# e-ago/CoMD-CUDA-Async

Hardware: AMD Instinct MI355X
Metric: atom_updates_per_sec (higher is better)
Workload: dtype f64

## Files before the change

### comd-cuda-async_amd/csrc/hip/comd_device.hip

```cpp
#include <hip/hip_runtime.h>
#include <cstdio>
#include <cstdlib>
#include <cstring>
#include <cmath>
#include <vector>
#include <map>
#include <utility>

#include "comd_hip.h"
#include "device_common.h"
#include "lj_kernels.h"
#include "lj_table_kernels.h"
#include "eam_kernels.h"
#include "step_kernels.h"
#include "nl_kernels.h"
#include "eam_brick_kernels.h"
#include "eam_atom_brick_kernels.h"
#include "virial_kernels.h"
#include "rdf_kernels.h"
#include "langevin_kernels.h"

static int g_rank = 0;

#define HIP_CHECK(cmd)                                                                                     \
   do {                                                                                                    \
      hipError_t status_ = (cmd);                                                                          \
      if (status_ != hipSuccess) {                                                                         \
         int dev_ = -1; (void)hipGetDevice(&dev_);                                                         \
         fprintf(stderr, "Rank %d, GPU: %d, Error in file %s at line %d\n", g_rank, dev_, __FILE__, __LINE__); \
         fprintf(stderr, "HIP error %d: %s\n", (int)status_, hipGetErrorString(status_));                  \
         exit(-1);                                                                                         \
      }                                                                                                    \
   } while (0)

#define LAUNCH_CHECK() HIP_CHECK(hipGetLastError())

static inline hipStream_t S(comdStream_t s) { return (hipStream_t)s; }
static inline int ceilDiv(long a, long b) { return (int)((a + b - 1) / b); }

static void allowDynamicLds(const void* fn, size_t lds)
{
   static std::map<std::pair<int, const void*>, size_t> granted;
   int dev = 0; HIP_CHECK(hipGetDevice(&dev));
   size_t& g = granted[std::make_pair(dev, fn)];
   if (lds > g) { HIP_CHECK(hipFuncSetAttribute(fn, hipFuncAttributeMaxDynamicSharedMemorySize, (int)lds)); g = lds; }
}

struct ComdTuning {
   bool   nlGlobal;
   bool   eamNlLds;
   int    ljWaves;
   bool   ljPrune;
   int    ljListCap;
   double ljListBudgetMb;
   bool   ljCtaSlabs;
   bool   eamCtaCell;
   bool   eamThreadAtomCell;
   bool   eamGroups;
   int    eamBrickBy, eamBrickBz;
   int    eamImage;
   int    eamAblate;
   bool   eamClamp;
   int    eamAtomRows;
   bool   eamAtomHandover;
   int    eamAtomBrickBy, eamAtomBrickBz;
   int    eamAtomLdsPad;
   int    eamCtaWaves;
   int    eamStencil;
   bool   nlSync;
   bool   eamListsEveryBuild;
   bool   nlBankOrder;
   double nlMargin;
};
static ComdTuning readTuning()
{
   auto env = getenv;
   auto num = [&](const char* name) { const char* e = env(name); return e ? atoi(e) : 0; };
   auto is = [&](const char* name, const char* value) { const char* e = env(name); return e && !strcmp(e, value); };
   auto isZero = [&](const char* name) { const char* e = env(name); return e && atoi(e) == 0; };
   auto shape = [&](const char* name, int* by, int* bz) { const char* e = env(name); if (!(e && sscanf(e, "%d,%d", by, bz) == 2 && *by >= 1 && *bz >= 1 && *by * *bz <= 64)) *by = *bz = 0; };
   ComdTuning t;
   t.nlGlobal = env("COMD_NL_GLOBAL") != nullptr;
   t.eamNlLds = is("COMD_EAM_NL", "lds");
   t.ljWaves = num("COMD_LJ_WAVES") > 0 ? num("COMD_LJ_WAVES") : 0;
   t.ljPrune = !isZero("COMD_LJ_PRUNE");
   t.ljListCap = num("COMD_LJ_LIST_CAP") > 0 ? (num("COMD_LJ_LIST_CAP") + 7) & ~7 : 0;
   t.ljListBudgetMb = env("COMD_LJ_LIST_BUDGET_MB") ? atof(env("COMD_LJ_LIST_BUDGET_MB")) : INFINITY;
   t.ljCtaSlabs = num("COMD_LJ_CTA_SLABS") != 0;
   t.eamCtaCell = is("COMD_EAM_CTA", "cell");
   t.eamThreadAtomCell = is("COMD_EAM_THREAD_ATOM", "cell");
   t.eamGroups = !isZero("COMD_EAM_GROUPS");
   shape("COMD_EAM_BRICK", &t.eamBrickBy, &t.eamBrickBz);
   t.eamImage = num("COMD_EAM_IMAGE") >= 64 ? (num("COMD_EAM_IMAGE") + 7) / 8 * 8 : 0;
   t.eamAblate = num("COMD_EAM_ABLATE");
   t.eamClamp = num("COMD_EAM_CLAMP") != 0;
   t.eamAtomRows = num("COMD_EAM_ATOM_ROWS") >= 8 && num("COMD_EAM_ATOM_ROWS") <= 128 ? num("COMD_EAM_ATOM_ROWS") / 8 * 8 : 0;
   t.eamAtomHandover = !isZero("COMD_EAM_ATOM_HANDOVER");
   shape("COMD_EAM_ATOM_BRICK", &t.eamAtomBrickBy, &t.eamAtomBrickBz);
   t.eamAtomLdsPad = num("COMD_EAM_ATOM_LDS_PAD");
   t.eamCtaWaves = num("COMD_EAM_CTA_WAVES") >= 1 && num("COMD_EAM_CTA_WAVES") <= 8 ? num("COMD_EAM_CTA_WAVES") : 0;
   t.eamStencil = num("COMD_EAM_STENCIL") >= 64 ? (num("COMD_EAM_STENCIL") + 7) / 8 * 8 : 0;
   t.nlSync = num("COMD_NL_SYNC") != 0;
   t.eamListsEveryBuild = env("COMD_EAM_LISTS_EVERY_BUILD") != nullptr;
   t.nlBankOrder = num("COMD_NL_BANK_ORDER") != 0;
   t.nlMargin = env("COMD_NL_MARGIN") && atof(env("COMD_NL_MARGIN")) >= 0.0 && atof(env("COMD_NL_MARGIN")) < 1.0 ? atof(env("COMD_NL_MARGIN")) : -1.0;
   return t;
}
static const ComdTuning& tuningOf(SimGpu* sim) { if (!sim->tuning) sim->tuning = new ComdTuning(readTuning()); return *(const ComdTuning*)sim->tuning; }
static double latticeConstantOf(const SimGpu* sim) { return sim->latticeConstant > 0.0 ? sim->latticeConstant : 3.615; }
static const double SPHERE_VOLUME = 4.18879020478639;


struct ForceTiming {
   struct Ev { hipEvent_t a, b; int kind; };
   std::vector<Ev> pool;
   size_t used = 0;
   double ms[2] = { 0.0, 0.0 };
   int launches[2] = { 0, 0 };
   bool on = false;
};

static void timingFlush(ForceTiming* t)
{
   if (!t) return;
   for (size_t i = 0; i < t->used; ++i) {
      float ms = 0.f;
      HIP_CHECK(hipEventSynchronize(t->pool[i].b));
      HIP_CHECK(hipEventElapsedTime(&ms, t->pool[i].a, t->pool[i].b));
      t->ms[t->pool[i].kind] += ms;
      t->launches[t->pool[i].kind] += 1;
   }
   t->used = 0;
}

struct ForceTimer {
   ForceTiming* t; hipStream_t st; int idx;
   ForceTimer(SimGpu* sim, hipStream_t s, int kind = 0) : t((ForceTiming*)sim->timing), st(s), idx(-1)
   {
// ... 368 lines not shown
{
   const size_t first = (size_t)sim->boxes.nLocalBoxes * sim->maxAtoms, slots = (size_t)(sim->boxes.nTotalBoxes - sim->boxes.nLocalBoxes) * sim->maxAtoms;
   const real_t* src[6] = { h->px, h->py, h->pz, h->rx, h->ry, h->rz };
   real_t* dst[6] = { sim->atoms.p.x, sim->atoms.p.y, sim->atoms.p.z, sim->atoms.r.x, sim->atoms.r.y, sim->atoms.r.z };
   for (int i = 0; i < 6; ++i) HIP_CHECK(hipMemcpy(dst[i] + first, src[i] + first, slots * sizeof(real_t), hipMemcpyHostToDevice));
   HIP_CHECK(hipMemcpy(sim->atoms.gid + first, h->gid + first, slots * sizeof(int), hipMemcpyHostToDevice));
   HIP_CHECK(hipMemcpy(sim->atoms.iSpecies + first, h->iSpecies + first, slots * sizeof(int), hipMemcpyHostToDevice));
}

extern "C" void updateNAtomsGpu(SimGpu* sim, const int* nAtomsHost)
{
   HIP_CHECK(hipMemcpy(sim->boxes.nAtoms, nAtomsHost, (size_t)sim->boxes.nTotalBoxes * sizeof(int), hipMemcpyHostToDevice));
}

extern "C" int compactHaloCells(const HostAtoms* h, int nLocalBoxes, int nTotalBoxes, int maxAtoms, char* h_compactAtoms, int* h_cellOffset)
{
   const int nHalo = nTotalBoxes - nLocalBoxes;
   h_cellOffset[0] = 0;
   for (int i = 0; i < nHalo; ++i) h_cellOffset[i + 1] = h_cellOffset[i] + h->nAtoms[nLocalBoxes + i];
   const int n = h_cellOffset[nHalo];
   int* gid = (int*)h_compactAtoms; int* type = gid + n;
   real_t* m = (real_t*)(type + n);
   for (int i = 0; i < nHalo; ++i) {
      size_t o = (size_t)(nLocalBoxes + i) * maxAtoms;
      for (int k = h_cellOffset[i]; k < h_cellOffset[i + 1]; ++k, ++o) {
         gid[k] = h->gid[o]; type[k] = h->iSpecies[o];
         m[k] = h->rx[o]; m[(size_t)n + k] = h->ry[o]; m[2 * (size_t)n + k] = h->rz[o];
         m[3 * (size_t)n + k] = h->px[o]; m[4 * (size_t)n + k] = h->py[o]; m[5 * (size_t)n + k] = h->pz[o];
      }
   }
   return n;
}

extern "C" void DestroyGpu(SimGpu* sim)
{
   HIP_CHECK(hipDeviceSynchronize());
   if (sim->timing) {
      ForceTiming* t = (ForceTiming*)sim->timing;
      timingFlush(t);
      for (auto& ev : t->pool) { (void)hipEventDestroy(ev.a); (void)hipEventDestroy(ev.b); }
      delete t;
   }
   delete (ComdTuning*)sim->tuning;
   void* ptrs[] = { sim->boxes.nAtoms, sim->atoms.r.x, sim->atoms.r.y, sim->atoms.r.z, sim->atoms.p.x, sim->atoms.p.y, sim->atoms.p.z,
                    sim->atoms.f.x, sim->atoms.f.y, sim->atoms.f.z, sim->atoms.e, sim->atoms.iSpecies, sim->atoms.gid,
                    sim->neighbor_cells, sim->species_mass, sim->eam_pot.phi.values, sim->eam_pot.rho.values, sim->eam_pot.f.values,
                    sim->eam_pot.rhobar, sim->eam_pot.dfEmbed, sim->nAtomsPrev, sim->cellDirty, sim->cellArrivals, sim->d_updateLinkCellsRequired, sim->status, sim->reduceBuf,
                    sim->boundary_cells, sim->interior_cells, sim->boundary1_cells,
                    sim->atoms.neighborList.list, sim->atoms.neighborList.nNeighbors, sim->atoms.neighborList.lastR.x,
                    sim->atoms.neighborList.lastR.y, sim->atoms.neighborList.lastR.z,
                    sim->atoms.neighborList.list16, sim->atoms.neighborList.stats, sim->atoms.neighborList.pairlist,
                    sim->boxes.boxIDLookUp, sim->boxes.boxIDLookUpReverse, sim->eam_pot.phiS.coefficients, sim->eam_pot.rhoS.coefficients,
                    sim->eam_pot.pairRows, sim->eam_pot.pairRowCount, sim->eam_pot.cellSel, sim->eam_pot.brickGroup, sim->eam_pot.brickList, sim->eam_pot.brickSel, sim->eam_pot.brickStats, sim->eam_pot.atomRows, sim->eam_pot.atomRowCount, sim->eam_pot.atomBrickSel,
                    sim->atoms.neighborList.brickRows, sim->atoms.neighborList.brickRowCount, sim->adapterScan, sim->lj_pot.waveCand, sim->lj_pot.waveCandCount, sim->lj_pot.packedR[0], sim->lj_pot.packedR[1], sim->lj_pot.packedF[0], sim->lj_pot.packedF[1],
                    sim->lj_pot.lj_interpolation.values, sim->virialBuf, sim->pairHistBuf };
   for (void* p : ptrs) if (p) HIP_CHECK(hipFree(p));
   if (sim->statusEvent) (void)hipEventDestroy((hipEvent_t)sim->statusEvent);
   if (sim->pinned) HIP_CHECK(hipHostFree(sim->pinned));
   if (sim->atoms.neighborList.updateRequiredHost) HIP_CHECK(hipHostFree(sim->atoms.neighborList.updateRequiredHost));
   if (sim->atoms.neighborList.brickStatsMirror) HIP_CHECK(hipHostFree(sim->atoms.neighborList.brickStatsMirror));
   if (sim->atoms.neighborList.brickStatsEvent) (void)hipEventDestroy((hipEvent_t)sim->atoms.neighborList.brickStatsEvent);
   if (sim->boundary_stream) HIP_CHECK(hipStreamDestroy(S(sim->boundary_stream)));
   if (sim->interior_stream) HIP_CHECK(hipStreamDestroy(S(sim->interior_stream)));
   memset(sim, 0, sizeof(*sim));
}

extern "C" void emptyHaloCellsGpu(SimGpu* sim, comdStream_t stream)
{
   const int nHalo = sim->boxes.nTotalBoxes - sim->boxes.nLocalBoxes;
   HIP_CHECK(hipMemsetAsync(sim->boxes.nAtoms + sim->boxes.nLocalBoxes, 0, (size_t)nHalo * sizeof(int), S(stream)));
}

extern "C" void comdCheckStatus(SimGpu* sim, const char* where)
{
   int st[4];
   HIP_CHECK(hipDeviceSynchronize());
   HIP_CHECK(hipMemcpy(st, sim->status, sizeof st, hipMemcpyDeviceToHost));
   if (st[0] | st[1] | st[2] | st[3]) {
      fprintf(stderr, "Rank %d, GPU: %d, %s: ", g_rank, sim->deviceId, where);
      if (st[0] & 1) fprintf(stderr, "a link cell overflowed its %d slots (raise --maxAtoms); ", sim->maxAtoms);
      if (st[0] & 2) fprintf(stderr, "a cell stencil holds more atoms than the cta_cell kernel can stage; ");
      if (st[1])     fprintf(stderr, "an atom moved beyond the halo region and was lost; ");
      if (st[2])     fprintf(stderr, "a halo message overflowed its buffer, or grew by more than 12.5 %% + 64 atoms in one step (COMD_HALO_HANDSHAKE=1 exchanges exact sizes); ");
      if (st[3] & 1) fprintf(stderr, "an atom has more neighbours inside the cutoff than a row of the EAM cta_cell kernel holds (1.5 x the FCC count; use -m thread_atom); ");
      if (st[3] & 2) fprintf(stderr, "an atom has more than %d neighbours inside cutoff + skin (raise --maxNeighbors); ", sim->atoms.neighborList.maxNeighbors);
      if (st[3] & 4) fprintf(stderr, "eamForce3Gpu[Async] covered the cells with another partition than eamForce1Gpu[Async] (include/comd_hip.h: same lists in both passes); ");
      fprintf(stderr, "\n");
      exit(-1);
   }
}

extern "C" void comdPollStatus(SimGpu* sim, comdStream_t stream, const char* where)
{
   int* mirror = (int*)(sim->pinned + 32);
   if (sim->statusMirrored) {
      sim->statusMirrored = 0;
      if (mirror[0] | mirror[1] | mirror[2] | mirror[3]) comdCheckStatus(sim, where);
      return;
   }
   if (sim->statusEvent) {
      if (hipEventQuery((hipEvent_t)sim->statusEvent) != hipSuccess) return;
      if (mirror[0] | mirror[1] | mirror[2] | mirror[3]) comdCheckStatus(sim, where);
   } else {
      hipEvent_t e; HIP_CHECK(hipEventCreateWithFlags(&e, hipEventDisableTiming)); sim->statusEvent = (void*)e;
   }
   HIP_CHECK(hipMemcpyAsync(mirror, sim->status, 4 * sizeof(int), hipMemcpyDeviceToHost, S(stream)));
   HIP_CHECK(hipEventRecord((hipEvent_t)sim->statusEvent, S(stream)));
}

extern "C" int comdReadDeviceInt(const int* d_ptr, comdStream_t stream)
{
   int v = 0;
   HIP_CHECK(hipMemcpyAsync(&v, d_ptr, sizeof(int), hipMemcpyDeviceToHost, S(stream)));
   HIP_CHECK(hipStreamSynchronize(S(stream)));
   return v;
}

static NlView nlView(SimGpu* sim)
{
   NeighborListGpu* n = &sim->atoms.neighborList;
   if (!n->list && !n->list16) { fprintf(stderr, "the *_nl methods need Verlet lists: allocate with GpuConfig.skinDistance > 0\n"); exit(-1); }
   if (n->nBuilds == 0) { fprintf(stderr, "the *_nl methods need buildNeighborListGpu before the first force call\n"); exit(-1); }
   NlView v; v.list = n->list; v.count = n->nNeighbors; v.maxNbr = n->maxNeighbors;
   return v;
}

static LjArgs makeLjArgs(SimGpu* sim, int num_cells, int* cells_list)
{
   LjArgs a;
   a.rx = sim->atoms.r.x; a.ry = sim->atoms.r.y; a.rz = sim->atoms.r.z;
   a.fx = sim->atoms.f.x; a.fy = sim->atoms.f.y; a.fz = sim->atoms.f.z; a.e = sim->atoms.e;
   a.nAtoms = sim->boxes.nAtoms; a.nbr = sim->neighbor_cells; a.cells = cells_list;
   a.nCells = num_cells; a.cap = sim->maxAtoms;
   const double sigma = sim->lj_pot.sigma, rc = sim->lj_pot.cutoff;
   a.rc2 = rc * rc;
   a.s6 = sigma * sigma * sigma * sigma * sigma * sigma;
   a.s6x2 = 2.0 * (sigma * sigma * sigma * sigma * sigma * sigma);
   const double rc6 = a.s6 / (a.rc2 * a.rc2 * a.rc2);
   a.eShift = rc6 * (rc6 - 1.0);
   a.eps = sim->lj_pot.epsilon;
   return a;
}

extern "C" void comdSetEnergyNeeded(SimGpu* sim, int on) { sim->needEnergy = on; }

static void ljBoxMargins(const SimGpu* sim, real_t rc2, real_t* rc2Box, real_t* grow)
{
   const double rel = sizeof(real_t) == 8 ? 1e-12 : 1e-5, eps = sizeof(real_t) == 8 ? 2.220446049250313e-16 : 1.1920929e-07;
   double big = 0.0;
   for (int a = 0; a < 3; ++a) {
      const double cellW = 1.0 / sim->boxes.invBoxSize[a];
      const double lo = fabs((double)sim->boxes.localMin[a] - cellW), hi = fabs((double)sim->boxes.localMax[a] + cellW);
      if (lo > big) big = lo;
      if (hi > big) big = hi;
   }
   const double rc = sqrt((double)rc2) * (1.0 + rel) + 8.0 * 1.7320508 * eps * big;
   *rc2Box = (real_t)(rc * rc);
   *grow = (real_t)(1.0 + rel);
}

static void ljBoxMarginsF(const SimGpu* sim, real_t rc2, float* rc2Box, float* grow)
{
   const double rel = 1e-5, eps = 1.1920929e-07;
   double big = 0.0;
   for (int a = 0; a < 3; ++a) {
      const double ext = (double)sim->boxes.localMax[a] - (double)sim->boxes.localMin[a] + 2.0 / sim->boxes.invBoxSize[a];
      if (ext > big) big = ext;
   }
   const double rc = sqrt((double)rc2) * (1.0 + rel) + 8.0 * 1.7320508 * eps * big;
   *rc2Box = (float)(rc * rc * (1.0 + 2.0 * eps));
   *grow = (float)(1.0 + rel);
}

struct LjThreadAtomLaunch { int w, wavesPerBlock; unsigned nBlocks; bool prune; LjWaveLists wl; };

static LjThreadAtomLaunch prepareLjThreadAtom(SimGpu* sim, const LjArgs& a, int num_cells, int* cells_list, comdStream_t stream)
{
   int w = sim->maxAtoms / 64;
   if (sim->max_atoms_cell > 0 && (sim->max_atoms_cell + 16 + 63) / 64 < w) w = (sim->max_atoms_cell + 16 + 63) / 64;
   const ComdTuning& tune = tuningOf(sim);
   if (tune.ljWaves && tune.ljWaves < w) w = tune.ljWaves;
   const int wavesPerBlock = w <= 4 ? w : 4;
   const unsigned nBlocks = w <= 4 ? (unsigned)num_cells : (unsigned)ceilDiv((long)num_cells * w, 4);
   const bool pruneEnv = tune.ljPrune;
   LjPotentialGpu* lj = &sim->lj_pot;
   if (pruneEnv && !lj->waveCand && lj->packedCap == 0) {
      std::vector<int> counts((size_t)sim->boxes.nTotalBoxes);
      HIP_CHECK(hipMemcpyAsync(counts.data(), sim->boxes.nAtoms, counts.size() * sizeof(int), hipMemcpyDeviceToHost, S(stream)));
      HIP_CHECK(hipStreamSynchronize(S(stream)));
      int fullest = sim->max_atoms_cell;
      for (int c : counts) if (c > fullest) fullest = c;
      const int occ = fullest + 16 < sim->maxAtoms ? fullest + 16 : sim->maxAtoms;
      lj->waveCandWaves = w;
      lj->waveCandCap = ((int)(0.70 * 27 * occ) + 7) & ~7;
      if (tune.ljListCap) lj->waveCandCap = tune.ljListCap;
      lj->packedCap = ((occ + 7) & ~7) < sim->maxAtoms ? ((occ + 7) & ~7) : sim->maxAtoms;
      const double listBytes = (double)sim->boxes.nLocalBoxes * lj->waveCandWaves * lj->waveCandCap * 4.0 + (double)sim->boxes.nLocalBoxes * lj->waveCandWaves * 8.0
                               + (sim->interior_stream ? 2.0 : 1.0) * (double)sim->boxes.nTotalBoxes * lj->packedCap * (sizeof(LjPos4) + sizeof(float4));
      size_t freeB = 0, totalB = 0;
      HIP_CHECK(hipMemGetInfo(&freeB, &totalB));
      if ((double)sim->boxes.nTotalBoxes * lj->packedCap * sizeof(LjPos4) >= 4294967296.0) lj->packedCap = -1;
      else if (listBytes + 2.0e9 > (double)freeB || listBytes > 1.0e6 * tune.ljListBudgetMb) {
         fprintf(stderr, "Rank %d: LJ candidate lists need %.1f GB, %.1f GB are free: running without them (the plain 27-cell walk, ~1.4x slower)\n",
                 g_rank, listBytes / 1e9, (double)freeB / 1e9);
         lj->packedCap = -1;
      } else {
         auto tryAlloc = [](size_t bytes) { void* p = nullptr; if (hipMalloc(&p, bytes ? bytes : 8) != hipSuccess) { (void)hipGetLastError(); p = nullptr; } return p; };
         const size_t recs = (size_t)sim->boxes.nTotalBoxes * lj->packedCap * 4;
         lj->waveCand = (unsigned*)tryAlloc((size_t)sim->boxes.nLocalBoxes * lj->waveCandWaves * lj->waveCandCap * sizeof(unsigned));
         lj->waveCandCount = (int*)tryAlloc((size_t)sim->boxes.nLocalBoxes * lj->waveCandWaves * 2 * sizeof(int));
         bool ok = lj->waveCand && lj->waveCandCount;
         for (int k = 0; k < (sim->interior_stream ? 2 : 1) && ok; ++k) {
            lj->packedR[k] = (real_t*)tryAlloc(recs * sizeof(real_t));
            lj->packedF[k] = (float*)tryAlloc(recs * sizeof(float));
            ok = lj->packedR[k] && lj->packedF[k];
         }
         if (!ok) {
            void* ps[6] = { lj->waveCand, lj->waveCandCount, lj->packedR[0], lj->packedF[0], lj->packedR[1], lj->packedF[1] };
            for (void* q : ps) if (q) (void)hipFree(q);
            lj->waveCand = nullptr; lj->waveCandCount = nullptr; lj->packedR[0] = lj->packedR[1] = nullptr; lj->packedF[0] = lj->packedF[1] = nullptr;
            fprintf(stderr, "Rank %d: the device refused the %.1f GB of the LJ candidate lists: running without them (the plain 27-cell walk, ~1.4x slower)\n", g_rank, listBytes / 1e9);
            lj->packedCap = -1;
         }
      }
   }
   const bool prune = pruneEnv && lj->waveCand;
   LjWaveLists wl; memset(&wl, 0, sizeof wl);
   if (prune) {
      const int which = (cells_list && stream != sim->interior_stream) ? 1 : 0;
      if (!lj->packedR[which]) {
         lj->packedR[which] = dalloc<real_t>((size_t)sim->boxes.nTotalBoxes * lj->packedCap * 4, false);
         lj->packedF[which] = dalloc<float>((size_t)sim->boxes.nTotalBoxes * lj->packedCap * 4, false);
      }
      wl.cand = lj->waveCand; wl.pos = (const LjPos4*)lj->packedR[which]; wl.posF = (const float4*)lj->packedF[which]; wl.count = (int2*)lj->waveCandCount;
      wl.candCap = lj->waveCandCap; wl.wavesMax = lj->waveCandWaves; wl.capP = lj->packedCap;
      ljBoxMarginsF(sim, a.rc2, &wl.rc2BoxF, &wl.growF);
      const int packCells = (cells_list && stream == sim->interior_stream) ? sim->boxes.nLocalBoxes : sim->boxes.nTotalBoxes;
      ForceTimer aux(sim, S(stream), 1);
      hipLaunchKernelGGL(LJ_PackPositions, dim3((unsigned)ceilDiv((long)packCells * lj->packedCap, 256)), dim3(256), 0, S(stream),
                         a.rx, a.ry, a.rz, a.nAtoms, (LjPos4*)lj->packedR[which], (float4*)lj->packedF[which], a.cap, lj->packedCap, packCells, a.rc2,
                         sim->boxes.localMin[0], sim->boxes.localMin[1], sim->boxes.localMin[2]);
      hipLaunchKernelGGL(LJ_WaveCandidates, dim3((unsigned)ceilDiv(num_cells, 4)), dim3(256), 0, S(stream), a, wl, w);
   }
   LjThreadAtomLaunch L; L.w = w; L.wavesPerBlock = wavesPerBlock; L.nBlocks = nBlocks; L.prune = prune; L.wl = wl;
   return L;
}

static TableView ljTableView(const SimGpu* sim)
{
   const InterpolationObjectGpu& t = sim->lj_pot.lj_interpolation;
   TableView tv; tv.v = t.values; tv.x0 = t.x0; tv.xn = t.xn; tv.invDx = t.invDx; tv.invDxHalf = t.invDxHalf; tv.invDxXx0 = t.invDxXx0;
   return tv;
}

static void launchLjThreadAtom(SimGpu* sim, const LjArgs& a, int num_cells, int* cells_list, comdStream_t stream, bool table)
{
   const LjThreadAtomLaunch L = prepareLjThreadAtom(sim, a, num_cells, cells_list, stream);
   const int w = L.w, wavesPerBlock = L.wavesPerBlock;
   const unsigned nBlocks = L.nBlocks;
   const bool prune = L.prune;
   const LjWaveLists& wl = L.wl;
   ForceTimer timer(sim, S(stream));
   if (table) {
      const TableView tv = ljTableView(sim);
#define LAUNCH_TABLE(E, LISTED) hipLaunchKernelGGL((LJ_Force_thread_atom_table<E, LISTED>), dim3(nBlocks), dim3(64 * wavesPerBlock), 0, S(stream), a, w, wl, tv)
      if (prune) { if (sim->needEnergy) LAUNCH_TABLE(true, true);  else LAUNCH_TABLE(false, true); }
      else       { if (sim->needEnergy) LAUNCH_TABLE(true, false); else LAUNCH_TABLE(false, false); }
#undef LAUNCH_TABLE
   } else if (prune) {
      if (sim->needEnergy) hipLaunchKernelGGL((LJ_Force_thread_atom<true, true>), dim3(nBlocks), dim3(64 * wavesPerBlock), 0, S(stream), a, w, wl);
      else              hipLaunchKernelGGL((LJ_Force_thread_atom<false, true>), dim3(nBlocks), dim3(64 * wavesPerBlock), 0, S(stream), a, w, wl);
   } else {
      if (sim->needEnergy) hipLaunchKernelGGL((LJ_Force_thread_atom<true, false>), dim3(nBlocks), dim3(64 * wavesPerBlock), 0, S(stream), a, w, wl);
      else              hipLaunchKernelGGL((LJ_Force_thread_atom<false, false>), dim3(nBlocks), dim3(64 * wavesPerBlock), 0, S(stream), a, w, wl);
   }
   LAUNCH_CHECK();
}

static void ljForce(SimGpu* sim, int num_cells, int* cells_list, int method, comdStream_t stream, bool table)
{
   if (num_cells <= 0) return;
   LjArgs a = makeLjArgs(sim, num_cells, cells_list);
   if (table) {
      if (!sim->lj_pot.lj_interpolation.values) { fprintf(stderr, "ljForceGpu: interpolation requested but there is no LJ table: call initLJinterpolation first\n"); exit(-1); }
      if (method == CTA_CELL) { fprintf(stderr, "ljForceGpu: interpolated LJ (-I) runs with thread_atom and thread_atom_nl, not cta_cell\n"); exit(-1); }
   }
   if (method != THREAD_ATOM_NL && method != WARP_ATOM_NL && method != CTA_CELL) { launchLjThreadAtom(sim, a, num_cells, cells_list, stream, table); return; }
   ForceTimer timer(sim, S(stream));
   if ((method == THREAD_ATOM_NL || method == WARP_ATOM_NL) && sim->atoms.neighborList.slabFormat) {
      NeighborListGpu* n = &sim->atoms.neighborList;
      (void)nlView(sim);
      NlSlabView v; v.list = n->list16; v.count = n->nNeighbors; v.rows = n->slabRows;
      const int threads = ((n->maxCellAtoms + 63) / 64) * 64;
// ... 689 lines not shown
```

### comd-cuda-async_amd/csrc/hip/lj_kernels.h

```cpp
#pragma once
#include "device_common.h"

struct LjArgs {
   const real_t* __restrict__ rx; const real_t* __restrict__ ry; const real_t* __restrict__ rz;
   real_t* __restrict__ fx; real_t* __restrict__ fy; real_t* __restrict__ fz; real_t* __restrict__ e;
   const int* __restrict__ nAtoms;
   const int* __restrict__ nbr;
   const int* __restrict__ cells;
   int nCells, cap;
   real_t rc2, s6, s6x2, eShift, eps;
};

template <bool ENERGY>
__device__ __forceinline__ void ljPair(real_t dx, real_t dy, real_t dz, real_t r2, const LjArgs& a,
                                       real_t& fx, real_t& fy, real_t& fz, real_t& e)
{
   const real_t ir2 = rcpR(r2);
   const real_t t = ir2 * ir2;
   const real_t w = t * ir2;
   if (ENERGY) { const real_t u = a.s6 * w; e += fmaR(u, u - R(1.0), -a.eShift); }
   const real_t fr = (t * t) * fmaR(w, a.s6x2, -R(1.0));
   fx = fmaR(fr, dx, fx); fy = fmaR(fr, dy, fy); fz = fmaR(fr, dz, fz);
}
#define LJ_FORCE_SCALE(a) (R(24.0) * (a).eps * (a).s6)

template <bool SELF, bool ENERGY>
__device__ __forceinline__ void ljCellLoop(const LjArgs& a, int jBox, real_t xi, real_t yi, real_t zi,
                                           real_t& fx, real_t& fy, real_t& fz, real_t& e)
{
   const int nj = uniform(a.nAtoms[jBox]);
   const real_t* __restrict__ px = a.rx + (size_t)jBox * a.cap;
   const real_t* __restrict__ py = a.ry + (size_t)jBox * a.cap;
   const real_t* __restrict__ pz = a.rz + (size_t)jBox * a.cap;
   int j = 0;
   for (; j + 8 <= nj; j += 8) {
      real_t xs[8], ys[8], zs[8];
#pragma unroll
      for (int u = 0; u < 8; ++u) { xs[u] = px[j + u]; ys[u] = py[j + u]; zs[u] = pz[j + u]; }
#pragma unroll
      for (int u = 0; u < 8; ++u) {
         real_t dx = xi - xs[u], dy = yi - ys[u], dz = zi - zs[u];
         real_t r2 = dx*dx + dy*dy + dz*dz;
         bool hit = SELF ? (r2 <= a.rc2 && r2 > R(0.0)) : (r2 <= a.rc2);
         if (hit) ljPair<ENERGY>(dx, dy, dz, r2, a, fx, fy, fz, e);
      }
   }
   for (; j < nj; ++j) {
      real_t dx = xi - px[j], dy = yi - py[j], dz = zi - pz[j];
      real_t r2 = dx*dx + dy*dy + dz*dz;
      bool hit = SELF ? (r2 <= a.rc2 && r2 > R(0.0)) : (r2 <= a.rc2);
      if (hit) ljPair<ENERGY>(dx, dy, dz, r2, a, fx, fy, fz, e);
   }
}

struct __attribute__((aligned(16))) LjPos4 { real_t x, y, z, rc2; };
struct LjWaveLists {
   unsigned* __restrict__ cand;
   const LjPos4* __restrict__ pos;
   int2*     __restrict__ count;
   int candCap, wavesMax;
   int capP;
   const float4* __restrict__ posF;
   float rc2BoxF, growF;
};

__device__ __forceinline__ LjPos4 atByte(const LjPos4* __restrict__ base, unsigned byteOff) { return *(const LjPos4*)((const char*)base + byteOff); }

template <bool SELF, bool ENERGY>
__device__ __forceinline__ void ljListTest(const LjArgs& a, const LjPos4& q, real_t xi, real_t yi, real_t zi, real_t& fx, real_t& fy, real_t& fz, real_t& e)
{
   real_t dx = xi - q.x, dy = yi - q.y, dz = zi - q.z;
   real_t r2 = dx*dx + dy*dy + dz*dz;
   bool hit = SELF ? (r2 <= q.rc2 && r2 > R(0.0)) : (r2 <= q.rc2);
   if (hit) ljPair<ENERGY>(dx, dy, dz, r2, a, fx, fy, fz, e);
}

template <bool SELF, bool ENERGY>
__device__ __forceinline__ void ljListLoop(const LjArgs& a, const LjPos4* __restrict__ pos, const unsigned* __restrict__ L, int p, int pEnd,
                                           real_t xi, real_t yi, real_t zi, real_t& fx, real_t& fy, real_t& fz, real_t& e)
{
   const int n8 = (pEnd - p) >> 3;
   if (n8 > 0) {
      const int last = p + 8 * (n8 - 1);
      unsigned id[8];
#pragma unroll
      for (int u = 0; u < 8; ++u) id[u] = L[p + u];
      for (int b = 0; b < n8; ++b, p += 8) {
         LjPos4 q[8];
         unsigned idn[8];
         const int pn = p + 8 < last ? p + 8 : last;
#pragma unroll
         for (int u = 0; u < 8; ++u) q[u] = atByte(pos, id[u]);
#pragma unroll
         for (int u = 0; u < 8; ++u) idn[u] = L[pn + u];
#pragma unroll
         for (int u = 0; u < 8; ++u) ljListTest<SELF, ENERGY>(a, q[u], xi, yi, zi, fx, fy, fz, e);
#pragma unroll
         for (int u = 0; u < 8; ++u) id[u] = idn[u];
      }
   }
   for (; p < pEnd; ++p) ljListTest<SELF, ENERGY>(a, atByte(pos, L[p]), xi, yi, zi, fx, fy, fz, e);
}

__global__ __launch_bounds__(256)
void LJ_PackPositions(const real_t* __restrict__ rx, const real_t* __restrict__ ry, const real_t* __restrict__ rz, const int* __restrict__ nAtoms,
                      LjPos4* __restrict__ pos, float4* __restrict__ posF, int cap, int capP, int nCells, real_t rc2, real_t ox, real_t oy, real_t oz)
{
   const long t = (long)blockIdx.x * blockDim.x + threadIdx.x;
   const int c = (int)(t / capP), i = (int)(t - (long)c * capP);
   if (c >= nCells || i >= nAtoms[c]) return;
   const size_t o = (size_t)c * cap + i;
   LjPos4 v; v.x = rx[o]; v.y = ry[o]; v.z = rz[o]; v.rc2 = rc2;
   pos[(size_t)c * capP + i] = v;
   posF[(size_t)c * capP + i] = make_float4((float)(v.x - ox), (float)(v.y - oy), (float)(v.z - oz), 0.0f);
}

__device__ __forceinline__ real_t waveMinR(real_t v) { for (int d = 1; d < 64; d <<= 1) v = minR(v, __shfl_xor(v, d)); return v; }
__device__ __forceinline__ real_t waveMaxR(real_t v) { for (int d = 1; d < 64; d <<= 1) v = maxR(v, __shfl_xor(v, d)); return v; }
#ifndef COMD_SINGLE
__device__ __forceinline__ float waveMinR(float v) { for (int d = 1; d < 64; d <<= 1) v = __builtin_fminf(v, __shfl_xor(v, d)); return v; }
__device__ __forceinline__ float waveMaxR(float v) { for (int d = 1; d < 64; d <<= 1) v = __builtin_fmaxf(v, __shfl_xor(v, d)); return v; }
#endif

__device__ __forceinline__ double uniformR(double v)
{
   const unsigned lo = (unsigned)__builtin_amdgcn_readfirstlane((int)(__double_as_longlong(v) & 0xffffffffll));
   const unsigned hi = (unsigned)__builtin_amdgcn_readfirstlane((int)(__double_as_longlong(v) >> 32));
   return __longlong_as_double((long long)(((unsigned long long)hi << 32) | lo));
}
__device__ __forceinline__ float uniformR(float v) { return __int_as_float(__builtin_amdgcn_readfirstlane(__float_as_int(v))); }

#define LJ_LIST_CHUNKS 4
#define LJ_LIST_TRIPS 3
#define LJ_LIST_BATCH 3
__global__ __launch_bounds__(256)
void LJ_WaveCandidates(LjArgs a, LjWaveLists w, int wavesPerCell)
{
   const int lane = threadIdx.x & 63;
   const int ci = uniform(blockIdx.x * (blockDim.x >> 6) + (threadIdx.x >> 6));
   if (ci >= a.nCells) return;
   const int iBox = uniform(a.cells ? a.cells[ci] : ci);
   const int ni = uniform(a.nAtoms[iBox]);
   int nChunks = (ni + 63) >> 6;
   if (nChunks > wavesPerCell) nChunks = wavesPerCell;
   if (nChunks > w.wavesMax) nChunks = w.wavesMax;
   if (nChunks <= 0) return;
   const int myBox = lane < 27 ? a.nbr[(size_t)iBox * 27 + lane] : 0;
   const int myCount = lane < 27 ? a.nAtoms[myBox] : 0;
   if (__ballot(myCount > w.capP) != 0ull) {
      if (lane < nChunks) w.count[iBox * w.wavesMax + lane] = make_int2(0, -1);
      return;
   }
   const float4* __restrict__ P = w.posF;
   const unsigned capP = (unsigned)w.capP;

   for (int c0 = 0; c0 < nChunks; c0 += LJ_LIST_CHUNKS) {
      float cx[LJ_LIST_CHUNKS], cy[LJ_LIST_CHUNKS], cz[LJ_LIST_CHUNKS], hx[LJ_LIST_CHUNKS], hy[LJ_LIST_CHUNKS], hz[LJ_LIST_CHUNKS];
      int n[LJ_LIST_CHUNKS], nSelf[LJ_LIST_CHUNKS];
#pragma unroll
      for (int c = 0; c < LJ_LIST_CHUNKS; ++c) {
         n[c] = 0; nSelf[c] = 0;
         cx[c] = cy[c] = cz[c] = hx[c] = hy[c] = hz[c] = 0.0f;
         if (c0 + c < nChunks) {
            const int iSlot = (c0 + c) * 64 + lane;
            const float4 q = P[(unsigned)iBox * capP + (unsigned)(iSlot < ni ? iSlot : ni - 1)];
            const float xlo = waveMinR(q.x), xhi = waveMaxR(q.x), ylo = waveMinR(q.y), yhi = waveMaxR(q.y), zlo = waveMinR(q.z), zhi = waveMaxR(q.z);
            cx[c] = uniformR(0.5f * (xlo + xhi)); hx[c] = uniformR(0.5f * (xhi - xlo) * w.growF);
            cy[c] = uniformR(0.5f * (ylo + yhi)); hy[c] = uniformR(0.5f * (yhi - ylo) * w.growF);
            cz[c] = uniformR(0.5f * (zlo + zhi)); hz[c] = uniformR(0.5f * (zhi - zlo) * w.growF);
         }
      }
      const int nC = nChunks - c0 < LJ_LIST_CHUNKS ? nChunks - c0 : LJ_LIST_CHUNKS;
      for (int k0 = 0; k0 < 27; k0 += LJ_LIST_BATCH) {
         float4 q[LJ_LIST_BATCH][LJ_LIST_TRIPS];
         int jb[LJ_LIST_BATCH], njb[LJ_LIST_BATCH];
#pragma unroll
         for (int b = 0; b < LJ_LIST_BATCH; ++b) {
            jb[b] = __builtin_amdgcn_readlane(myBox, k0 + b); njb[b] = __builtin_amdgcn_readlane(myCount, k0 + b);
#pragma unroll
            for (int t = 0; t < LJ_LIST_TRIPS; ++t) {
               const int j = 64 * t + lane;
               if (64 * t < njb[b]) q[b][t] = P[(unsigned)jb[b] * capP + (unsigned)(j < njb[b] ? j : 0)];
            }
         }
#pragma unroll
         for (int b = 0; b < LJ_LIST_BATCH; ++b) {
            const int njNow = njb[b];
            const unsigned base = (unsigned)jb[b] * capP;
            for (int j0 = 0; j0 < njNow; j0 += 64 * LJ_LIST_TRIPS) {
               if (j0 > 0) {
#pragma unroll
                  for (int t = 0; t < LJ_LIST_TRIPS; ++t) {
                     const int j = j0 + 64 * t + lane;
                     q[b][t] = P[base + (unsigned)(j < njNow ? j : 0)];
                  }
               }
#pragma unroll
               for (int t = 0; t < LJ_LIST_TRIPS; ++t) {
                  const int rem = njNow - (j0 + 64 * t);
                  if (rem <= 0) break;
                  const unsigned long long valid = rem >= 64 ? ~0ull : (1ull << rem) - 1ull;
                  const unsigned entry = (base + (unsigned)(j0 + 64 * t + lane)) * (unsigned)sizeof(LjPos4);
#pragma unroll
                  for (int c = 0; c < LJ_LIST_CHUNKS; ++c) {
                     if (c >= nC) break;
                     const float dx = __builtin_fmaxf(0.0f, __builtin_fabsf(q[b][t].x - cx[c]) - hx[c]);
                     const float dy = __builtin_fmaxf(0.0f, __builtin_fabsf(q[b][t].y - cy[c]) - hy[c]);
                     const float dz = __builtin_fmaxf(0.0f, __builtin_fabsf(q[b][t].z - cz[c]) - hz[c]);
                     const unsigned long long mask = __ballot(dx*dx + dy*dy + dz*dz <= w.rc2BoxF) & valid;
                     const unsigned pos = __builtin_amdgcn_mbcnt_hi((unsigned)(mask >> 32), __builtin_amdgcn_mbcnt_lo((unsigned)mask, (unsigned)n[c]));
                     char* __restrict__ L = (char*)(w.cand + (size_t)(iBox * w.wavesMax + c0 + c) * w.candCap);
                     if (__builtin_amdgcn_inverse_ballot_w64(mask) && pos < (unsigned)w.candCap) *(unsigned*)(L + (pos << 2)) = entry;
                     n[c] += __popcll(mask);
                  }
               }
            }
            if (k0 + b == 0) {
#pragma unroll
               for (int c = 0; c < LJ_LIST_CHUNKS; ++c) nSelf[c] = n[c];
            }
         }
      }
#pragma unroll
      for (int c = 0; c < LJ_LIST_CHUNKS; ++c)
         if (c0 + c < nChunks && lane == 0) w.count[iBox * w.wavesMax + c0 + c] = n[c] <= w.candCap ? make_int2(nSelf[c], n[c]) : make_int2(0, -1);
   }
}

template <bool ENERGY>
__device__ __forceinline__ void ljChunkGeneric(const LjArgs& a, int iBox, int ni, int chunk, int lane)
{
   const int* __restrict__ nb = a.nbr + (size_t)iBox * 27;
   const int m = ni - chunk * 64 < 64 ? ni - chunk * 64 : 64;
   const int G = 64 / m < 4 ? 64 / m : 4;
   const int g = lane / m, ai = lane - g * m;
   const bool valid = g < G;
   const size_t iOff = (size_t)iBox * a.cap + chunk * 64 + (valid ? ai : 0);
   const real_t xi = a.rx[iOff], yi = a.ry[iOff], zi = a.rz[iOff];
   real_t fx = R(0.0), fy = R(0.0), fz = R(0.0), e = R(0.0);
   for (int t = 0; t * G < 27; ++t) {
      const int k = t * G + g;
      const bool okk = valid && k < 27;
      const int jBox = okk ? nb[k] : iBox;
      const int nj = okk ? a.nAtoms[jBox] : 0;
      const size_t base = (size_t)jBox * a.cap;
      for (int j = 0; __any(j < nj); ++j) {
         if (j < nj) {
            const real_t dx = xi - a.rx[base + j], dy = yi - a.ry[base + j], dz = zi - a.rz[base + j];
            const real_t r2 = dx*dx + dy*dy + dz*dz;
            if (r2 <= a.rc2 && r2 > R(0.0)) ljPair<ENERGY>(dx, dy, dz, r2, a, fx, fy, fz, e);
         }
      }
   }
   real_t tx = fx, ty = fy, tz = fz, te = e;
   for (int r = 1; r < G; ++r) {
      const int src = (ai + r * m) & 63;
      tx += bpermuteR(fx, src); ty += bpermuteR(fy, src); tz += bpermuteR(fz, src);
      if (ENERGY) te += bpermuteR(e, src);
   }
   if (lane < m) {
      const real_t fs = LJ_FORCE_SCALE(a);
      a.fx[iOff] = tx * fs; a.fy[iOff] = ty * fs; a.fz[iOff] = tz * fs;
      if (ENERGY) a.e[iOff] = te * R(2.0) * a.eps;
   }
// ... 338 lines not shown
```

### include/comd_hip.h

```cpp
#ifndef COMD_HIP_H
#define COMD_HIP_H

#include <stdint.h>

#ifdef __cplusplus
extern "C" {
#endif

#ifndef __MYTYPE_H_
#ifdef COMD_SINGLE
typedef float real_t;
#else
typedef double real_t;
#endif
typedef struct vec_t { real_t* x; real_t* y; real_t* z; } vec_t;
#endif
typedef void*  comdStream_t;

#ifndef __DEFINES_H_
enum { THREAD_ATOM = 0, THREAD_ATOM_NL = 1, WARP_ATOM = 2, WARP_ATOM_NL = 3, CTA_CELL = 4, CPU_NL = 5 };
#endif

typedef struct InterpolationObjectGpuSt {
   int     n;
   real_t  x0, xn, invDx, invDxHalf, invDxXx0;
   real_t* values;
} InterpolationObjectGpu;

typedef struct LjPotentialGpuSt {
   real_t cutoff, sigma, epsilon;
   unsigned* waveCand;
   int*      waveCandCount;
   int       waveCandCap, waveCandWaves;
   int       packedCap;
   real_t*   packedR[2];
   float*    packedF[2];
   InterpolationObjectGpu lj_interpolation;
} LjPotentialGpu;

typedef struct InterpolationSplineObjectGpuSt {
   int     n;
   float   x0, xn, invDx, invDxXx0;
   real_t* coefficients;
} InterpolationSplineObjectGpu;

typedef struct EamPotentialGpuSt {
   real_t cutoff;
   InterpolationObjectGpu phi, rho, f;
   InterpolationSplineObjectGpu phiS, rhoS;
   real_t* rhobar;
   real_t* dfEmbed;
   unsigned* pairRows;
   unsigned short* pairRowCount;
   int     pairRowLen;
   int     brickImageCap;
   int*    brickGroup;
   int     brickGroupBy, brickGroupBz;
   int*    brickList;
   int     brickCount[2], brickListStride;
   int     brickListMakes;
   int     brickListsValid;
   int     brickCountAll;
   int*    cellSel;
   int     selTag;
   unsigned long long* brickSel;
   int*    brickStats;
   int     brickBy, brickBz;
   int     atomBrickBy, atomBrickBz;
   int     atomBrickImageCap;
   unsigned* atomRows;
   unsigned short* atomRowCount;
   unsigned long long* atomBrickSel;
   int     atomRowsValid;
} EamPotentialGpu;

typedef struct LinkCellGpuSt {
   int    nLocalBoxes, nTotalBoxes;
   int    gridSize[3];
   real_t localMin[3], localMax[3], invBoxSize[3];
   int*   nAtoms;
   int*   boxIDLookUp;
   int*   boxIDLookUpReverse;
} LinkCellGpu;

typedef struct NeighborListGpuSt {
   int*   list;
   int*   nNeighbors;
   int    maxNeighbors;
   vec_t  lastR;
// ... 263 lines not shown
```

Baseline: 671.5 million.

## Precompute per-chunk bounding boxes and classify chunk pairs to skip LJ candidate tests

The pack kernel now computes a per-64-atom chunk bounding box along with the packed positions. The candidate-list kernel loads these boxes instead of reducing them per wave. It classifies each (i-chunk, j-chunk) pair as beyond, inside or straddling the cutoff. Beyond pairs are skipped and inside pairs are appended wholesale without per-atom tests, which avoids loads and ballots. The change adds extra memory, a launch-shape change for packing and an occupancy hint (waves_per_eu), and risks correctness through the in/out margin computations.

```diff
diff --git a/comd-cuda-async_amd/csrc/hip/comd_device.hip b/comd-cuda-async_amd/csrc/hip/comd_device.hip
--- a/comd-cuda-async_amd/csrc/hip/comd_device.hip
+++ b/comd-cuda-async_amd/csrc/hip/comd_device.hip
@@ -51,6 +51,7 @@
    bool   eamNlLds;
    int    ljWaves;
    bool   ljPrune;
+   bool   ljListChunkBox;
    int    ljListCap;
    double ljListBudgetMb;
    bool   ljCtaSlabs;
@@ -84,6 +85,7 @@
    t.eamNlLds = is("COMD_EAM_NL", "lds");
    t.ljWaves = num("COMD_LJ_WAVES") > 0 ? num("COMD_LJ_WAVES") : 0;
    t.ljPrune = !isZero("COMD_LJ_PRUNE");
+   t.ljListChunkBox = !isZero("COMD_LJ_LIST_CHUNKBOX");
    t.ljListCap = num("COMD_LJ_LIST_CAP") > 0 ? (num("COMD_LJ_LIST_CAP") + 7) & ~7 : 0;
    t.ljListBudgetMb = env("COMD_LJ_LIST_BUDGET_MB") ? atof(env("COMD_LJ_LIST_BUDGET_MB")) : INFINITY;
    t.ljCtaSlabs = num("COMD_LJ_CTA_SLABS") != 0;
@@ -558,7 +560,7 @@
                     sim->atoms.neighborList.list16, sim->atoms.neighborList.stats, sim->atoms.neighborList.pairlist,
                     sim->boxes.boxIDLookUp, sim->boxes.boxIDLookUpReverse, sim->eam_pot.phiS.coefficients, sim->eam_pot.rhoS.coefficients,
                     sim->eam_pot.pairRows, sim->eam_pot.pairRowCount, sim->eam_pot.cellSel, sim->eam_pot.brickGroup, sim->eam_pot.brickList, sim->eam_pot.brickSel, sim->eam_pot.brickStats, sim->eam_pot.atomRows, sim->eam_pot.atomRowCount, sim->eam_pot.atomBrickSel,
-                    sim->atoms.neighborList.brickRows, sim->atoms.neighborList.brickRowCount, sim->adapterScan, sim->lj_pot.waveCand, sim->lj_pot.waveCandCount, sim->lj_pot.packedR[0], sim->lj_pot.packedR[1], sim->lj_pot.packedF[0], sim->lj_pot.packedF[1],
+                    sim->atoms.neighborList.brickRows, sim->atoms.neighborList.brickRowCount, sim->adapterScan, sim->lj_pot.waveCand, sim->lj_pot.waveCandCount, sim->lj_pot.packedR[0], sim->lj_pot.packedR[1], sim->lj_pot.packedF[0], sim->lj_pot.packedF[1], sim->lj_pot.chunkBoxF[0], sim->lj_pot.chunkBoxF[1],
                     sim->lj_pot.lj_interpolation.values, sim->virialBuf, sim->pairHistBuf };
    for (void* p : ptrs) if (p) HIP_CHECK(hipFree(p));
    if (sim->statusEvent) (void)hipEventDestroy((hipEvent_t)sim->statusEvent);
@@ -665,7 +667,7 @@
    *grow = (real_t)(1.0 + rel);
 }
 
-static void ljBoxMarginsF(const SimGpu* sim, real_t rc2, float* rc2Box, float* grow)
+static void ljBoxMarginsF(const SimGpu* sim, real_t rc2, float* rc2Box, float* grow, float* rc2In = nullptr, float* rc2Out = nullptr)
 {
    const double rel = 1e-5, eps = 1.1920929e-07;
    double big = 0.0;
@@ -676,6 +678,9 @@
    const double rc = sqrt((double)rc2) * (1.0 + rel) + 8.0 * 1.7320508 * eps * big;
    *rc2Box = (float)(rc * rc * (1.0 + 2.0 * eps));
    *grow = (float)(1.0 + rel);
+   const double m = rc - sqrt((double)rc2);
+   if (rc2In) *rc2In = (float)((double)rc2 * (1.0 - 2.0 * eps));
+   if (rc2Out) *rc2Out = (float)((rc + m) * (rc + m) * (1.0 + 2.0 * eps));
 }
 
 struct LjThreadAtomLaunch { int w, wavesPerBlock; unsigned nBlocks; bool prune; LjWaveLists wl; };
@@ -702,7 +707,7 @@
       if (tune.ljListCap) lj->waveCandCap = tune.ljListCap;
       lj->packedCap = ((occ + 7) & ~7) < sim->maxAtoms ? ((occ + 7) & ~7) : sim->maxAtoms;
       const double listBytes = (double)sim->boxes.nLocalBoxes * lj->waveCandWaves * lj->waveCandCap * 4.0 + (double)sim->boxes.nLocalBoxes * lj->waveCandWaves * 8.0
-                               + (sim->interior_stream ? 2.0 : 1.0) * (double)sim->boxes.nTotalBoxes * lj->packedCap * (sizeof(LjPos4) + sizeof(float4));
+                               + (sim->interior_stream ? 2.0 : 1.0) * (double)sim->boxes.nTotalBoxes * (lj->packedCap * (sizeof(LjPos4) + sizeof(float4)) + ceilDiv(lj->packedCap, 64) * 2.0 * sizeof(float4));
       size_t freeB = 0, totalB = 0;
       HIP_CHECK(hipMemGetInfo(&freeB, &totalB));
       if ((double)sim->boxes.nTotalBoxes * lj->packedCap * sizeof(LjPos4) >= 4294967296.0) lj->packedCap = -1;
@@ -713,18 +718,20 @@
       } else {
          auto tryAlloc = [](size_t bytes) { void* p = nullptr; if (hipMalloc(&p, bytes ? bytes : 8) != hipSuccess) { (void)hipGetLastError(); p = nullptr; } return p; };
          const size_t recs = (size_t)sim->boxes.nTotalBoxes * lj->packedCap * 4;
+         const size_t boxes = (size_t)sim->boxes.nTotalBoxes * ceilDiv(lj->packedCap, 64) * 8;
          lj->waveCand = (unsigned*)tryAlloc((size_t)sim->boxes.nLocalBoxes * lj->waveCandWaves * lj->waveCandCap * sizeof(unsigned));
          lj->waveCandCount = (int*)tryAlloc((size_t)sim->boxes.nLocalBoxes * lj->waveCandWaves * 2 * sizeof(int));
          bool ok = lj->waveCand && lj->waveCandCount;
          for (int k = 0; k < (sim->interior_stream ? 2 : 1) && ok; ++k) {
             lj->packedR[k] = (real_t*)tryAlloc(recs * sizeof(real_t));
             lj->packedF[k] = (float*)tryAlloc(recs * sizeof(float));
-            ok = lj->packedR[k] && lj->packedF[k];
+            lj->chunkBoxF[k] = (float*)tryAlloc(boxes * sizeof(float));
+            ok = lj->packedR[k] && lj->packedF[k] && lj->chunkBoxF[k];
          }
          if (!ok) {
-            void* ps[6] = { lj->waveCand, lj->waveCandCount, lj->packedR[0], lj->packedF[0], lj->packedR[1], lj->packedF[1] };
+            void* ps[8] = { lj->waveCand, lj->waveCandCount, lj->packedR[0], lj->packedF[0], lj->packedR[1], lj->packedF[1], lj->chunkBoxF[0], lj->chunkBoxF[1] };
             for (void* q : ps) if (q) (void)hipFree(q);
-            lj->waveCand = nullptr; lj->waveCandCount = nullptr; lj->packedR[0] = lj->packedR[1] = nullptr; lj->packedF[0] = lj->packedF[1] = nullptr;
+            lj->waveCand = nullptr; lj->waveCandCount = nullptr; lj->packedR[0] = lj->packedR[1] = nullptr; lj->packedF[0] = lj->packedF[1] = nullptr; lj->chunkBoxF[0] = lj->chunkBoxF[1] = nullptr;
             fprintf(stderr, "Rank %d: the device refused the %.1f GB of the LJ candidate lists: running without them (the plain 27-cell walk, ~1.4x slower)\n", g_rank, listBytes / 1e9);
             lj->packedCap = -1;
          }
@@ -737,14 +744,16 @@
       if (!lj->packedR[which]) {
          lj->packedR[which] = dalloc<real_t>((size_t)sim->boxes.nTotalBoxes * lj->packedCap * 4, false);
          lj->packedF[which] = dalloc<float>((size_t)sim->boxes.nTotalBoxes * lj->packedCap * 4, false);
+         lj->chunkBoxF[which] = dalloc<float>((size_t)sim->boxes.nTotalBoxes * ceilDiv(lj->packedCap, 64) * 8, false);
       }
       wl.cand = lj->waveCand; wl.pos = (const LjPos4*)lj->packedR[which]; wl.posF = (const float4*)lj->packedF[which]; wl.count = (int2*)lj->waveCandCount;
       wl.candCap = lj->waveCandCap; wl.wavesMax = lj->waveCandWaves; wl.capP = lj->packedCap;
-      ljBoxMarginsF(sim, a.rc2, &wl.rc2BoxF, &wl.growF);
+      wl.boxF = (const float4*)lj->chunkBoxF[which]; wl.chunksP = ceilDiv(lj->packedCap, 64); wl.chunkBox = tune.ljListChunkBox ? 1 : 0;
+      ljBoxMarginsF(sim, a.rc2, &wl.rc2BoxF, &wl.growF, &wl.rc2InF, &wl.rc2OutF);
       const int packCells = (cells_list && stream == sim->interior_stream) ? sim->boxes.nLocalBoxes : sim->boxes.nTotalBoxes;
       ForceTimer aux(sim, S(stream), 1);
-      hipLaunchKernelGGL(LJ_PackPositions, dim3((unsigned)ceilDiv((long)packCells * lj->packedCap, 256)), dim3(256), 0, S(stream),
-                         a.rx, a.ry, a.rz, a.nAtoms, (LjPos4*)lj->packedR[which], (float4*)lj->packedF[which], a.cap, lj->packedCap, packCells, a.rc2,
+      hipLaunchKernelGGL(LJ_PackPositions, dim3((unsigned)ceilDiv((long)packCells * wl.chunksP, 4)), dim3(256), 0, S(stream),
+                         a.rx, a.ry, a.rz, a.nAtoms, (LjPos4*)lj->packedR[which], (float4*)lj->packedF[which], (float4*)lj->chunkBoxF[which], a.cap, lj->packedCap, wl.chunksP, packCells, a.rc2,
                          sim->boxes.localMin[0], sim->boxes.localMin[1], sim->boxes.localMin[2]);
       hipLaunchKernelGGL(LJ_WaveCandidates, dim3((unsigned)ceilDiv(num_cells, 4)), dim3(256), 0, S(stream), a, wl, w);
    }
diff --git a/comd-cuda-async_amd/csrc/hip/lj_kernels.h b/comd-cuda-async_amd/csrc/hip/lj_kernels.h
--- a/comd-cuda-async_amd/csrc/hip/lj_kernels.h
+++ b/comd-cuda-async_amd/csrc/hip/lj_kernels.h
@@ -62,6 +62,10 @@
    int capP;
    const float4* __restrict__ posF;
    float rc2BoxF, growF;
+   const float4* __restrict__ boxF;
+   int chunksP;
+   int chunkBox;
+   float rc2InF, rc2OutF;
 };
 
 __device__ __forceinline__ LjPos4 atByte(const LjPos4* __restrict__ base, unsigned byteOff) { return *(const LjPos4*)((const char*)base + byteOff); }
@@ -100,19 +104,6 @@
       }
    }
    for (; p < pEnd; ++p) ljListTest<SELF, ENERGY>(a, atByte(pos, L[p]), xi, yi, zi, fx, fy, fz, e);
-}
-
-__global__ __launch_bounds__(256)
-void LJ_PackPositions(const real_t* __restrict__ rx, const real_t* __restrict__ ry, const real_t* __restrict__ rz, const int* __restrict__ nAtoms,
-                      LjPos4* __restrict__ pos, float4* __restrict__ posF, int cap, int capP, int nCells, real_t rc2, real_t ox, real_t oy, real_t oz)
-{
-   const long t = (long)blockIdx.x * blockDim.x + threadIdx.x;
-   const int c = (int)(t / capP), i = (int)(t - (long)c * capP);
-   if (c >= nCells || i >= nAtoms[c]) return;
-   const size_t o = (size_t)c * cap + i;
-   LjPos4 v; v.x = rx[o]; v.y = ry[o]; v.z = rz[o]; v.rc2 = rc2;
-   pos[(size_t)c * capP + i] = v;
-   posF[(size_t)c * capP + i] = make_float4((float)(v.x - ox), (float)(v.y - oy), (float)(v.z - oz), 0.0f);
 }
 
 __device__ __forceinline__ real_t waveMinR(real_t v) { for (int d = 1; d < 64; d <<= 1) v = minR(v, __shfl_xor(v, d)); return v; }
@@ -122,6 +113,37 @@
 __device__ __forceinline__ float waveMaxR(float v) { for (int d = 1; d < 64; d <<= 1) v = __builtin_fmaxf(v, __shfl_xor(v, d)); return v; }
 #endif
 
+#define LJ_EMPTY_HALF (-1.0e30f)
+__global__ __launch_bounds__(256)
+void LJ_PackPositions(const real_t* __restrict__ rx, const real_t* __restrict__ ry, const real_t* __restrict__ rz, const int* __restrict__ nAtoms,
+                      LjPos4* __restrict__ pos, float4* __restrict__ posF, float4* __restrict__ boxF, int cap, int capP, int chunksP, int nCells,
+                      real_t rc2, real_t ox, real_t oy, real_t oz)
+{
+   const int lane = threadIdx.x & 63;
+   const int gw = uniform(blockIdx.x * (blockDim.x >> 6) + (threadIdx.x >> 6));
+   const int c = gw / chunksP, chunk = gw - c * chunksP;
+   if (c >= nCells) return;
+   int n = uniform(nAtoms[c]);
+   if (n > capP) n = capP;
+   const int first = chunk * 64;
+   float4* __restrict__ B = boxF + ((size_t)c * chunksP + chunk) * 2;
+   if (first >= n) {
+      if (lane == 0) { B[0] = make_float4(0.0f, 0.0f, 0.0f, 0.0f); B[1] = make_float4(LJ_EMPTY_HALF, LJ_EMPTY_HALF, LJ_EMPTY_HALF, 0.0f); }
+      return;
+   }
+   const int i = first + lane;
+   const bool live = i < n;
+   const size_t o = (size_t)c * cap + (live ? i : first);
+   LjPos4 v; v.x = rx[o]; v.y = ry[o]; v.z = rz[o]; v.rc2 = rc2;
+   const float4 f = make_float4((float)(v.x - ox), (float)(v.y - oy), (float)(v.z - oz), 0.0f);
+   if (live) { pos[(size_t)c * capP + i] = v; posF[(size_t)c * capP + i] = f; }
+   const float xlo = waveMinR(f.x), xhi = waveMaxR(f.x), ylo = waveMinR(f.y), yhi = waveMaxR(f.y), zlo = waveMinR(f.z), zhi = waveMaxR(f.z);
+   if (lane == 0) {
+      B[0] = make_float4(0.5f * (xlo + xhi), 0.5f * (ylo + yhi), 0.5f * (zlo + zhi), 0.0f);
+      B[1] = make_float4(0.5f * (xhi - xlo), 0.5f * (yhi - ylo), 0.5f * (zhi - zlo), 0.0f);
+   }
+}
+
 __device__ __forceinline__ double uniformR(double v)
 {
    const unsigned lo = (unsigned)__builtin_amdgcn_readfirstlane((int)(__double_as_longlong(v) & 0xffffffffll));
@@ -133,7 +155,10 @@
 #define LJ_LIST_CHUNKS 4
 #define LJ_LIST_TRIPS 3
 #define LJ_LIST_BATCH 3
-__global__ __launch_bounds__(256)
+#define LJ_CHUNK_BEYOND 0u
+#define LJ_CHUNK_INSIDE 1u
+#define LJ_CHUNK_STRADDLE 2u
+__global__ __launch_bounds__(256) __attribute__((amdgpu_waves_per_eu(6, 8)))
 void LJ_WaveCandidates(LjArgs a, LjWaveLists w, int wavesPerCell)
 {
    const int lane = threadIdx.x & 63;
@@ -153,34 +178,58 @@
    }
    const float4* __restrict__ P = w.posF;
    const unsigned capP = (unsigned)w.capP;
-
    for (int c0 = 0; c0 < nChunks; c0 += LJ_LIST_CHUNKS) {
+      float4 bc[2], bh[2];
+      bool has[2];
+   #pragma unroll
+      for (int s = 0; s < 2; ++s) {
+         const int f = 64 * s + lane;
+         const int k = f / LJ_LIST_TRIPS < 27 ? f / LJ_LIST_TRIPS : 26, t = f - (f / LJ_LIST_TRIPS) * LJ_LIST_TRIPS;
+         const int jBox = __shfl(myBox, k), nj = __shfl(myCount, k);
+         has[s] = f < 27 * LJ_LIST_TRIPS && 64 * t < nj;
+         bc[s] = bh[s] = make_float4(0.0f, 0.0f, 0.0f, 0.0f);
+         if (has[s]) { const float4* __restrict__ B = w.boxF + ((size_t)jBox * w.chunksP + t) * 2; bc[s] = B[0]; bh[s] = B[1]; }
+      }
       float cx[LJ_LIST_CHUNKS], cy[LJ_LIST_CHUNKS], cz[LJ_LIST_CHUNKS], hx[LJ_LIST_CHUNKS], hy[LJ_LIST_CHUNKS], hz[LJ_LIST_CHUNKS];
       int n[LJ_LIST_CHUNKS], nSelf[LJ_LIST_CHUNKS];
+      const int nC = nChunks - c0 < LJ_LIST_CHUNKS ? nChunks - c0 : LJ_LIST_CHUNKS;
+      unsigned cls[2] = { 0u, 0u };
 #pragma unroll
       for (int c = 0; c < LJ_LIST_CHUNKS; ++c) {
          n[c] = 0; nSelf[c] = 0;
          cx[c] = cy[c] = cz[c] = hx[c] = hy[c] = hz[c] = 0.0f;
          if (c0 + c < nChunks) {
-            const int iSlot = (c0 + c) * 64 + lane;
-            const float4 q = P[(unsigned)iBox * capP + (unsigned)(iSlot < ni ? iSlot : ni - 1)];
-            const float xlo = waveMinR(q.x), xhi = waveMaxR(q.x), ylo = waveMinR(q.y), yhi = waveMaxR(q.y), zlo = waveMinR(q.z), zhi = waveMaxR(q.z);
-            cx[c] = uniformR(0.5f * (xlo + xhi)); hx[c] = uniformR(0.5f * (xhi - xlo) * w.growF);
-            cy[c] = uniformR(0.5f * (ylo + yhi)); hy[c] = uniformR(0.5f * (yhi - ylo) * w.growF);
-            cz[c] = uniformR(0.5f * (zlo + zhi)); hz[c] = uniformR(0.5f * (zhi - zlo) * w.growF);
-         }
-      }
-      const int nC = nChunks - c0 < LJ_LIST_CHUNKS ? nChunks - c0 : LJ_LIST_CHUNKS;
+            const float4* __restrict__ B = w.boxF + ((size_t)iBox * w.chunksP + (c0 + c)) * 2;
+            const float4 oc = B[0], oh = B[1];
+            cx[c] = uniformR(oc.x); hx[c] = uniformR(oh.x * w.growF);
+            cy[c] = uniformR(oc.y); hy[c] = uniformR(oh.y * w.growF);
+            cz[c] = uniformR(oc.z); hz[c] = uniformR(oh.z * w.growF);
+#pragma unroll
+            for (int s = 0; s < 2; ++s) {
+               const float ax = __builtin_fabsf(bc[s].x - cx[c]) - hx[c], ay = __builtin_fabsf(bc[s].y - cy[c]) - hy[c], az = __builtin_fabsf(bc[s].z - cz[c]) - hz[c];
+               const float gx = __builtin_fmaxf(0.0f, ax - bh[s].x * w.growF), gy = __builtin_fmaxf(0.0f, ay - bh[s].y * w.growF), gz = __builtin_fmaxf(0.0f, az - bh[s].z * w.growF);
+               const float fx = __builtin_fmaxf(0.0f, ax + bh[s].x), fy = __builtin_fmaxf(0.0f, ay + bh[s].y), fz = __builtin_fmaxf(0.0f, az + bh[s].z);
+               unsigned k = LJ_CHUNK_STRADDLE;
+               if (w.chunkBox) {
+                  if (gx*gx + gy*gy + gz*gz > w.rc2OutF) k = LJ_CHUNK_BEYOND;
+                  else if (fx*fx + fy*fy + fz*fz <= w.rc2InF) k = LJ_CHUNK_INSIDE;
+               }
+               if (has[s]) cls[s] |= k << (2 * c);
+            }
+         }
+      }
+      const unsigned allStraddle = 0xAAu & ((1u << (2 * nC)) - 1u);
       for (int k0 = 0; k0 < 27; k0 += LJ_LIST_BATCH) {
          float4 q[LJ_LIST_BATCH][LJ_LIST_TRIPS];
          int jb[LJ_LIST_BATCH], njb[LJ_LIST_BATCH];
+         auto classesOf = [&](int k, int t) { const int f = k * LJ_LIST_TRIPS + t; return (unsigned)(f < 64 ? __builtin_amdgcn_readlane((int)cls[0], f) : __builtin_amdgcn_readlane((int)cls[1], f - 64)); };
 #pragma unroll
          for (int b = 0; b < LJ_LIST_BATCH; ++b) {
             jb[b] = __builtin_amdgcn_readlane(myBox, k0 + b); njb[b] = __builtin_amdgcn_readlane(myCount, k0 + b);
 #pragma unroll
             for (int t = 0; t < LJ_LIST_TRIPS; ++t) {
                const int j = 64 * t + lane;
-               if (64 * t < njb[b]) q[b][t] = P[(unsigned)jb[b] * capP + (unsigned)(j < njb[b] ? j : 0)];
+               if (classesOf(k0 + b, t) & 0xAAu) q[b][t] = P[(unsigned)jb[b] * capP + (unsigned)(j < njb[b] ? j : 0)];
             }
          }
 #pragma unroll
@@ -199,17 +248,26 @@
                for (int t = 0; t < LJ_LIST_TRIPS; ++t) {
                   const int rem = njNow - (j0 + 64 * t);
                   if (rem <= 0) break;
+                  const unsigned classes = j0 == 0 ? classesOf(k0 + b, t) : allStraddle;
                   const unsigned long long valid = rem >= 64 ? ~0ull : (1ull << rem) - 1ull;
                   const unsigned entry = (base + (unsigned)(j0 + 64 * t + lane)) * (unsigned)sizeof(LjPos4);
 #pragma unroll
                   for (int c = 0; c < LJ_LIST_CHUNKS; ++c) {
                      if (c >= nC) break;
+                     const unsigned k = (classes >> (2 * c)) & 3u;
+                     if (k == LJ_CHUNK_BEYOND) continue;
+                     char* __restrict__ L = (char*)(w.cand + (size_t)(iBox * w.wavesMax + c0 + c) * w.candCap);
+                     if (k == LJ_CHUNK_INSIDE) {
+                        const unsigned pos = (unsigned)n[c] + (unsigned)lane;
+                        if (lane < rem && pos < (unsigned)w.candCap) *(unsigned*)(L + (pos << 2)) = entry;
+                        n[c] += rem < 64 ? rem : 64;
+                        continue;
+                     }
                      const float dx = __builtin_fmaxf(0.0f, __builtin_fabsf(q[b][t].x - cx[c]) - hx[c]);
                      const float dy = __builtin_fmaxf(0.0f, __builtin_fabsf(q[b][t].y - cy[c]) - hy[c]);
                      const float dz = __builtin_fmaxf(0.0f, __builtin_fabsf(q[b][t].z - cz[c]) - hz[c]);
                      const unsigned long long mask = __ballot(dx*dx + dy*dy + dz*dz <= w.rc2BoxF) & valid;
                      const unsigned pos = __builtin_amdgcn_mbcnt_hi((unsigned)(mask >> 32), __builtin_amdgcn_mbcnt_lo((unsigned)mask, (unsigned)n[c]));
-                     char* __restrict__ L = (char*)(w.cand + (size_t)(iBox * w.wavesMax + c0 + c) * w.candCap);
                      if (__builtin_amdgcn_inverse_ballot_w64(mask) && pos < (unsigned)w.candCap) *(unsigned*)(L + (pos << 2)) = entry;
                      n[c] += __popcll(mask);
                   }
diff --git a/include/comd_hip.h b/include/comd_hip.h
--- a/include/comd_hip.h
+++ b/include/comd_hip.h
@@ -35,6 +35,7 @@
    int       packedCap;
    real_t*   packedR[2];
    float*    packedF[2];
+   float*    chunkBoxF[2];
    InterpolationObjectGpu lj_interpolation;
 } LjPotentialGpu;
 
```

Result: slower. 650.6 million (-3.1%).
